# darchr/EmbeddingTables.jl

Measured on AMD Instinct MI355X. Metric: embedding lookups/sec + achieved HBM GB/s (% of roofline), 26 tables x dim128 at B=65536, higher is better.
Workload: dtype f32

## Files before the change

embeddingtables.jl_amd/csrc/et_lookup.hip:

```cpp
#include <type_traits>
#include "et_common.h"

#include <stdlib.h>
#include <string.h>

#include <mutex>
#include <utility>
#include <vector>

namespace et {

struct XcdQueue;
struct LookupPack {
    et_lookup_desc d[ET_MAX_TABLES_PER_LAUNCH];
    XcdQueue* queue = nullptr;
};

template <typename T, int D>
struct VecGeom {
    static constexpr int N = 16 / (int)sizeof(T);
    static constexpr int VPR = D / N;
    static constexpr int LPR = VPR < 64 ? VPR : 64;
    static constexpr int NV = VPR / LPR;
    static constexpr int GPW = 64 / LPR;
    static constexpr int U = NV >= 8 ? 1 : 8 / NV;
    static_assert(D % N == 0, "row must be whole vectors");
    static_assert(VPR <= 64 ? (64 % VPR == 0) : (VPR % 64 == 0), "unsupported row size");
};

template <typename T, int N>
__device__ __forceinline__ void unpack16(u32x4 v, T (&x)[N]) {
    static_assert(N * sizeof(T) == 16, "");
    __builtin_memcpy(x, &v, 16);
}

template <typename T, int N>
__device__ __forceinline__ u32x4 pack16(const T (&x)[N]) {
    u32x4 v;
    __builtin_memcpy(&v, x, 16);
    return v;
}

constexpr int kBcastReadlaneMaxGpw = 2;
template <int LPR>
__device__ __forceinline__ long long group_bcast(long long v, int i, int g) {
    constexpr int GPW = 64 / LPR;
    if constexpr (GPW <= kBcastReadlaneMaxGpw) {
        const int lo = (int)v, hi = (int)(v >> 32);
        int rlo = __builtin_amdgcn_readlane(lo, i), rhi = __builtin_amdgcn_readlane(hi, i);
#pragma unroll
        for (int gg = 1; gg < GPW; ++gg) {
            const int tlo = __builtin_amdgcn_readlane(lo, gg * LPR + i);
            const int thi = __builtin_amdgcn_readlane(hi, gg * LPR + i);
            rlo = g == gg ? tlo : rlo;
            rhi = g == gg ? thi : rhi;
        }
        return (long long)(((unsigned long long)(unsigned)rhi << 32) | (unsigned)rlo);
    } else {
        return __shfl(v, g * LPR + i, 64);
    }
}

template <int LPR>
__device__ __forceinline__ uint32_t group_bcast32(uint32_t v, int i, int g) {
    constexpr int GPW = 64 / LPR;
    if constexpr (GPW <= kBcastReadlaneMaxGpw) {
        int r = __builtin_amdgcn_readlane((int)v, i);
#pragma unroll
        for (int gg = 1; gg < GPW; ++gg) {
            const int t = __builtin_amdgcn_readlane((int)v, gg * LPR + i);
            r = g == gg ? t : r;
        }
        return (uint32_t)r;
    } else {
        return (uint32_t)__shfl((int)v, g * LPR + i, 64);
    }
}

__device__ __forceinline__ uint32_t idx_row32(long long v, uint32_t nrows) {
    const uint64_t row = (uint64_t)(v - 1);
    return row < (uint64_t)nrows ? (uint32_t)row : ~0u;
}

template <int LPR>
__device__ __forceinline__ long long load_idx_chunk(const int64_t* __restrict__ ip, int cnt,
                                                    int sub) {
    return (long long)ip[sub < cnt ? sub : cnt - 1];
}

template <typename T, typename A, int D, int UU, bool NTL, bool PG = false, bool MK = false>
__device__ __forceinline__ void load_add(const T* __restrict__ table, uint32_t ld_table,
                                         uint32_t nrows, uint32_t cpp, uint32_t myr, int g,
                                         int sub, int i0, bool first_batch,
                                         A (&acc)[VecGeom<T, D>::NV][VecGeom<T, D>::N],
                                         int& bad, int vpr) {
    using G = VecGeom<T, D>;
    constexpr int N = G::N, LPR = G::LPR, NV = G::NV;
    uint64_t off[UU];
    bool ok[UU];
    const T* base[UU];
#pragma unroll
    for (int u = 0; u < UU; ++u) {
        const uint32_t r = group_bcast32<LPR>(myr, i0 + u, g);
        ok[u] = r != ~0u;
        const uint32_t row32 = ok[u] ? r : 0u;
        if constexpr (PG) {
            const uint32_t page = row32 / cpp;
            off[u] = (uint64_t)(row32 - page * cpp) * ld_table;
            base[u] = reinterpret_cast<const T* const*>(table)[page];
        } else {
            off[u] = (uint64_t)row32 * ld_table;
            base[u] = table;
        }
    }
    int vix[NV];
#pragma unroll
    for (int v = 0; v < NV; ++v) {
        vix[v] = sub + v * LPR;
        if constexpr (MK) vix[v] = vix[v] < vpr ? vix[v] : vpr - 1;
    }
    u32x4 buf[UU][NV];
#pragma unroll
    for (int u = 0; u < UU; ++u) {
        const u32x4* src = reinterpret_cast<const u32x4*>(base[u] + off[u]);
#pragma unroll
        for (int v = 0; v < NV; ++v) {
            if constexpr (NTL)
                buf[u][v] = __builtin_nontemporal_load(src + vix[v]);
            else
                buf[u][v] = src[vix[v]];
        }
    }
    int anybad = 0;
#pragma unroll
    for (int u = 0; u < UU; ++u) anybad |= ok[u] ? 0 : 1;
    auto add_rows = [&](auto checked) {
#pragma unroll
        for (int u = 0; u < UU; ++u) {
#pragma unroll
            for (int v = 0; v < NV; ++v) {
                T x[N];
                if constexpr (decltype(checked)::value)
                    unpack16<T, N>(ok[u] ? buf[u][v] : u32x4{0u, 0u, 0u, 0u}, x);
                else
                    unpack16<T, N>(buf[u][v], x);
#pragma unroll
                for (int k = 0; k < N; ++k) {
                    if (u == 0)
                        acc[v][k] = first_batch ? A(x[k]) : A(acc[v][k] + A(x[k]));
                    else
                        acc[v][k] = A(acc[v][k] + A(x[k]));
                }
            }
        }
    };
    if (__builtin_expect(__any(anybad), 0)) {
#pragma unroll
        for (int u = 0; u < UU; ++u) bad += ok[u] ? 0 : 1;
        add_rows(std::true_type{});
    } else {
        add_rows(std::false_type{});
    }
}

template <typename T, typename A, int D, int U, bool NT, bool NTL, bool PG = false,
          bool MK = false>
__device__ __forceinline__ void bag_sum_vec(const T* __restrict__ table, uint32_t ld_table,
                                            uint32_t nrows, uint32_t cpp,
                                            const int64_t* __restrict__ ip,
                                            int pool, long long my0, T* __restrict__ out, int g,
                                            int sub, int vpr) {
    using G = VecGeom<T, D>;
    constexpr int N = G::N, LPR = G::LPR, NV = G::NV;
    A acc[NV][N];
#pragma unroll
    for (int v = 0; v < NV; ++v)
#pragma unroll
        for (int k = 0; k < N; ++k) acc[v][k] = A(0);
    int bad = 0;

    for (int c0 = 0; c0 < pool; c0 += LPR) {
        const int cnt = pool - c0 < LPR ? pool - c0 : LPR;
        const long long my = c0 == 0 ? my0 : load_idx_chunk<LPR>(ip + c0, cnt, sub);
        const uint32_t myr = idx_row32(my, nrows);
        int i0 = 0;
#define ET_LOAD_ADD(UU) \
    load_add<T, A, D, UU, NTL, PG, MK>(table, ld_table, nrows, cpp, myr, g, sub, i0,       \
                                       c0 + i0 == 0, acc, bad, vpr)
        for (; i0 + U <= cnt; i0 += U) ET_LOAD_ADD(U);
        if constexpr (U > 8) {
            if (cnt - i0 >= 8) {
                ET_LOAD_ADD(8);
                i0 += 8;
            }
        }
        if constexpr (U > 4) {
            if (cnt - i0 >= 4) {
                ET_LOAD_ADD(4);
                i0 += 4;
            }
        }
        if constexpr (U > 2) {
            if (cnt - i0 >= 2) {
                ET_LOAD_ADD(2);
                i0 += 2;
            }
        }
        if (cnt - i0 >= 1) ET_LOAD_ADD(1);
#undef ET_LOAD_ADD
    }
    if (bad && sub == 0) note_oob(bad);
    u32x4* o = reinterpret_cast<u32x4*>(out) + sub;
#pragma unroll
    for (int v = 0; v < NV; ++v) {
        T y[N];
#pragma unroll
        for (int k = 0; k < N; ++k) y[k] = T(acc[v][k]);
        if (!MK || sub + v * LPR < vpr) store16<NT>(o + v * LPR, pack16<T, N>(y));
    }
}

template <typename T, typename A, int D, int U, bool NT, bool NTL, bool PG = false,
          bool MK = false>
__device__ __forceinline__ void run_bags(const et_lookup_desc& d, int64_t batch,
                                         T* __restrict__ dst, int64_t ld_dst, int64_t chunk,
                                         int rounds) {
    using G = VecGeom<T, D>;
    const T* table = reinterpret_cast<const T*>(d.table);
    const int lane = threadIdx.x & 63, wave = threadIdx.x >> 6;
    const int g = lane / G::LPR, sub = lane % G::LPR;
    const int64_t per_round = 4 * G::GPW;
    const int pool = d.pool;
    const int cnt0 = pool < G::LPR ? pool : G::LPR;
    const uint32_t ldt = (uint32_t)d.ld_table, nr = (uint32_t)d.nrows;
    const int vpr = MK ? d.dim / G::N : G::VPR;
    int64_t bag = chunk * per_round * rounds + wave * G::GPW + g;
    long long my_next = load_idx_chunk<G::LPR>(
        d.idx + (bag < batch ? bag : batch - 1) * d.ld_idx, cnt0, sub);
    for (int r = 0; r < rounds; ++r) {
        if (bag >= batch) break;
        const long long my = my_next;
        const int64_t nbag = bag + per_round;
        if (r + 1 < rounds)
            my_next = load_idx_chunk<G::LPR>(
                d.idx + (nbag < batch ? nbag : batch - 1) * d.ld_idx, cnt0, sub);
        bag_sum_vec<T, A, D, U, NT, NTL, PG, MK>(table, ldt, nr, (uint32_t)d.cols_per_page,
                                                 d.idx + bag * d.ld_idx, pool, my,
                                                 dst + bag * ld_dst + d.dst_row_off, g, sub, vpr);
        bag = nbag;
    }
}

typedef const __attribute__((address_space(4))) int64_t* cidx_ptr;

__device__ __forceinline__ cidx_ptr as_scalar_idx(const int64_t* p) {
    return (cidx_ptr)(uintptr_t)p;
}

__device__ __forceinline__ uint64_t row_off_s(int64_t v, uint32_t ldb, uint32_t nrows,
                                              uint32_t& bad) {
    const uint32_t lo = (uint32_t)v - 1u;
    const uint32_t borrow = (uint32_t)(((uint64_t)lo - (uint64_t)nrows) >> 32);
    bad |= (uint32_t)((uint64_t)v >> 32) | ~borrow;
    return (((uint64_t)__umulhi(lo, ldb)) << 32) | (uint64_t)(lo * ldb);
}

template <typename T, typename A, int UU, bool NTL>
__device__ __forceinline__ bool load_add_s(uintptr_t tb, uint32_t ldb, uint32_t nrows,
                                           cidx_ptr ia, cidx_ptr ib, uint64_t hmask,
                                           uint64_t lane_off, bool first_batch,
                                           A (&acc)[16 / sizeof(T)]) {
    constexpr int N = 16 / (int)sizeof(T);
    typedef const __attribute__((address_space(1))) u32x4 gvec;
    uint64_t oa[UU], dd[UU];
    uint32_t bad = 0u;
#pragma unroll
    for (int u = 0; u < UU; ++u) {
        oa[u] = row_off_s(ia[u], ldb, nrows, bad);
        dd[u] = row_off_s(ib[u], ldb, nrows, bad) - oa[u];
    }
    if (bad) return false;
    u32x4 buf[UU];
#pragma unroll
    for (int u = 0; u < UU; ++u) {
        const uint64_t a = ((dd[u] & hmask) + lane_off) + (tb + oa[u]);
        const gvec* src = reinterpret_cast<const gvec*>(a);
        if constexpr (NTL)
            buf[u] = __builtin_nontemporal_load(src);
        else
            buf[u] = *src;
    }
#pragma unroll
    for (int u = 0; u < UU; ++u) {
        T x[N];
        __builtin_memcpy(x, &buf[u], 16);
#pragma unroll
        for (int k = 0; k < N; ++k) {
            if (u == 0)
                acc[k] = first_batch ? A(x[k]) : A(acc[k] + A(x[k]));
            else
                acc[k] = A(acc[k] + A(x[k]));
        }
    }
    return true;
}

template <typename T, typename A>
__device__ __forceinline__ void bag_pair_checked(uintptr_t tb, uint32_t ldb, uint32_t nrows,
                                                 const int64_t* ia, const int64_t* ib, bool hi,
                                                 int sub, int pool, A* acc, int* bad) {
    constexpr int N = 16 / (int)sizeof(T);
    const int64_t* ip = hi ? ib : ia;
#pragma unroll 1
    for (int i = 0; i < pool; ++i) {
        const uint64_t r = (uint64_t)(ip[i] - 1);
        const bool ok = r < (uint64_t)nrows;
        *bad += ok ? 0 : 1;
        const u32x4 v = *(reinterpret_cast<const u32x4*>(
                              tb + (uint64_t)(ok ? (uint32_t)r : 0u) * ldb) + sub);
        T x[N];
        unpack16<T, N>(ok ? v : u32x4{0u, 0u, 0u, 0u}, x);
        for (int k = 0; k < N; ++k) acc[k] = i == 0 ? A(x[k]) : A(acc[k] + A(x[k]));
    }
}

template <typename T, typename A, int U, bool NT, bool NTL>
__device__ __forceinline__ void run_bags_s(const et_lookup_desc& d, int64_t batch,
                                           T* __restrict__ dst, int64_t ld_dst, int64_t chunk,
                                           int rounds) {
    constexpr int N = 16 / (int)sizeof(T);
    const int lane = threadIdx.x & 63;
    const int wave = __builtin_amdgcn_readfirstlane(threadIdx.x >> 6);
    const bool hi = lane >= 32;
    const int sub = lane & 31;
    uint32_t hm = hi ? ~0u : 0u;
    asm volatile("" : "+v"(hm));
    const uint64_t hmask = ((uint64_t)hm << 32) | hm, lane_off = (uint64_t)sub * 16u;
    const uintptr_t tb = reinterpret_cast<uintptr_t>(d.table);
    const uint32_t ldb = (uint32_t)(d.ld_table * (int64_t)sizeof(T)), nr = (uint32_t)d.nrows;
    const int pool = d.pool;
    int64_t bag = chunk * 8 * rounds + 2 * wave;
    for (int r = 0; r < rounds; ++r, bag += 8) {
        if (bag >= batch) break;
        const bool has_b = bag + 1 < batch;
        const cidx_ptr ia = as_scalar_idx(d.idx + bag * d.ld_idx);
        const cidx_ptr ib = has_b ? as_scalar_idx(d.idx + (bag + 1) * d.ld_idx) : ia;
        A acc[N];
#pragma unroll
        for (int k = 0; k < N; ++k) acc[k] = A(0);
        bool ok = true;
        int i0 = 0;
#define ET_LOAD_ADD_S(UU) \
    load_add_s<T, A, UU, NTL>(tb, ldb, nr, ia + i0, ib + i0, hmask, lane_off, i0 == 0, acc)
        for (; ok && i0 + U <= pool; i0 += U) ok = ET_LOAD_ADD_S(U);
        if constexpr (U > 4) {
            if (ok && pool - i0 >= 4) {
                ok = ET_LOAD_ADD_S(4);
                i0 += 4;
            }
        }
        if constexpr (U > 2) {
            if (ok && pool - i0 >= 2) {
                ok = ET_LOAD_ADD_S(2);
                i0 += 2;
            }
        }
        if (ok && pool - i0 >= 1) ok = ET_LOAD_ADD_S(1);
#undef ET_LOAD_ADD_S
        int bad = 0;
        if (!ok)
            bag_pair_checked<T, A>(tb, ldb, nr, d.idx + bag * d.ld_idx,
                                   d.idx + (has_b ? bag + 1 : bag) * d.ld_idx, hi, sub, pool, acc,
                                   &bad);
        if (hi && !has_b) bad = 0;
        if (bad && sub == 0) note_oob(bad);
        if (!hi || has_b) {
            T y[N];
#pragma unroll
            for (int k = 0; k < N; ++k) y[k] = T(acc[k]);
            u32x4* o =
                reinterpret_cast<u32x4*>(dst + (bag + (hi ? 1 : 0)) * ld_dst + d.dst_row_off) + sub;
            store16<NT>(o, pack16<T, N>(y));
        }
    }
}

template <typename T, typename A, int D, int U, bool NT, bool PG = false, bool MK = false,
          bool SG = false>
__global__ __launch_bounds__(256) void k_pooled_vec(LookupPack pack, int ntables, int64_t batch,
                                                    T* __restrict__ dst, int64_t ld_dst,
                                                    int rounds) {
    const int64_t item = blockIdx.x;
    const int t = (int)(item % ntables);
    const int64_t chunk = item / ntables;
    if constexpr (SG)
        run_bags_s<T, A, U, NT, false>(pack.d[t], batch, dst, ld_dst, chunk, rounds);
    else
        run_bags<T, A, D, U, NT, false, PG, MK>(pack.d[t], batch, dst, ld_dst, chunk, rounds);
}

constexpr int kXcds = 8;

constexpr int kMaxStripeEntries = 40;
struct StripeMap {
    uint32_t entry[kXcds][kMaxStripeEntries];
    int nent;
    uint32_t ntload_mask;
    uint32_t prio_mask;
    int nheavy;
    int affinity;
    int fab_share;
};

template <typename T, typename A, int D, int U, bool NT, bool SG>
__device__ __forceinline__ void striped_body(const LookupPack& pack, const StripeMap& sm,
                                             int ntables, int64_t batch, T* __restrict__ dst,
                                             int64_t ld_dst, int rounds, int64_t stripe_chunks,
                                             int64_t nchunks, int x = blockIdx.x % kXcds,
                                             int64_t slot = blockIdx.x / kXcds) {
    const int k = (int)(slot % ntables);
    const int64_t j = slot / ntables;
    const uint32_t e = sm.entry[x][k];
    const int t = (int)(e & 0xff);
    const int64_t chunk = (int64_t)((e >> 8) & 0xff) * stripe_chunks + j;
    if (j >= stripe_chunks || chunk >= nchunks) return;
    if ((sm.prio_mask >> t) & 1u) __builtin_amdgcn_s_setprio(2);
    if constexpr (SG) {
        if ((sm.ntload_mask >> t) & 1u)
            run_bags_s<T, A, U, NT, true>(pack.d[t], batch, dst, ld_dst, chunk, rounds);
        else
            run_bags_s<T, A, U, NT, false>(pack.d[t], batch, dst, ld_dst, chunk, rounds);
    } else {
        if ((sm.ntload_mask >> t) & 1u)
            run_bags<T, A, D, U, NT, true>(pack.d[t], batch, dst, ld_dst, chunk, rounds);
        else
            run_bags<T, A, D, U, NT, false>(pack.d[t], batch, dst, ld_dst, chunk, rounds);
    }
}

#ifdef ET_WG_TIMELINE
constexpr uint32_t kTlCap = 1u << 17;
__device__ uint4 g_tl[kTlCap][2];
#endif

__device__ __forceinline__ uint64_t tl_begin() {
#ifdef ET_WG_TIMELINE
    return __builtin_amdgcn_s_memrealtime();
#else
    return 0;
#endif
}

__device__ __forceinline__ void tl_stamp(uint64_t t0, const StripeMap& sm, int ntables,
                                         int64_t stripe_chunks, int64_t nchunks, int x,
                                         int64_t slot) {
#ifdef ET_WG_TIMELINE
    __syncthreads();
    if (threadIdx.x == 0 && blockIdx.x < kTlCap) {
        const uint64_t t1 = __builtin_amdgcn_s_memrealtime();
        uint32_t xcc, hw;
        asm volatile("s_getreg_b32 %0, hwreg(HW_REG_XCC_ID)" : "=s"(xcc));
        asm volatile("s_getreg_b32 %0, hwreg(HW_REG_HW_ID)" : "=s"(hw));
        uint32_t t = 0xffu;
        if (x >= 0) {
            const int64_t j = slot / ntables;
            const uint32_t e = sm.entry[x][slot % ntables];
            const int64_t chunk = (int64_t)((e >> 8) & 0xff) * stripe_chunks + j;
            t = (j >= stripe_chunks || chunk >= nchunks ? 0xffu : (e & 0xffu)) | ((uint32_t)x << 8);
        }
        g_tl[blockIdx.x][0] = make_uint4((uint32_t)t0, (uint32_t)(t0 >> 32), (uint32_t)t1,
                                         (uint32_t)(t1 >> 32));
        g_tl[blockIdx.x][1] = make_uint4(t, xcc, hw, gridDim.x);
    }
#endif
}

template <typename T, typename A, int D, int U, bool NT, bool SG = false>
__global__ __launch_bounds__(256) void k_pooled_vec_striped(LookupPack pack, StripeMap sm,
                                                            int ntables, int64_t batch,
                                                            T* __restrict__ dst, int64_t ld_dst,
                                                            int rounds, int64_t stripe_chunks,
                                                            int64_t nchunks) {
    const uint64_t t0 = tl_begin();
    striped_body<T, A, D, U, NT, SG>(pack, sm, ntables, batch, dst, ld_dst, rounds, stripe_chunks,
                                     nchunks);
    tl_stamp(t0, sm, ntables, stripe_chunks, nchunks, blockIdx.x % kXcds, blockIdx.x / kXcds);
}

struct XcdQueue {
    uint32_t head[kXcds][2];
    uint32_t done;
    uint32_t pad[32 - 2 * kXcds - 1];
};
static_assert(sizeof(XcdQueue) == ET_LOOKUP_QUEUE_BYTES, "queue block size (include/embtab.h)");

__device__ __forceinline__ uint32_t cu_hash16(uint32_t hw) {
    const uint32_t cu = (hw >> 8) & 15u, sh = (hw >> 12) & 1u, se = (hw >> 13) & 7u;
    const uint32_t v = (cu + 3u * se + 5u * sh) & 15u;
    return ((v & 1u) << 3) | ((v & 2u) << 1) | ((v & 4u) >> 1) | ((v & 8u) >> 3);
}

__device__ __forceinline__ uint32_t claim_class(XcdQueue& q, uint32_t x, uint32_t c,
                                                uint32_t nheavy, uint32_t ntables, uint32_t sc) {
    const uint32_t nk = c ? ntables - nheavy : nheavy;
    const uint32_t h = atomicAdd(&q.head[x][c], 1u);
    if (h >= nk * sc) return ~0u;
    return x * (ntables * sc) + (h / nk) * ntables + (c ? nheavy : 0u) + h % nk;
}

__device__ __forceinline__ uint32_t claim_pref(XcdQueue& q, uint32_t x0, uint32_t p,
                                               uint32_t nheavy, uint32_t ntables, uint32_t sc) {
    constexpr uint32_t M = (uint32_t)(kXcds - 1);
    uint32_t it = claim_class(q, x0, p, nheavy, ntables, sc);
    if (it == ~0u && p == 1u) it = claim_class(q, x0, 0u, nheavy, ntables, sc);
    for (uint32_t k = 1; it == ~0u && k < (uint32_t)kXcds; ++k)
        it = claim_class(q, (x0 + k) & M, 0u, nheavy, ntables, sc);
    if (it == ~0u && p == 0u) it = claim_class(q, x0, 1u, nheavy, ntables, sc);
    for (uint32_t k = 1; it == ~0u && k < (uint32_t)kXcds; ++k)
        it = claim_class(q, (x0 + k) & M, 1u, nheavy, ntables, sc);
    return it;
}

template <typename T, typename A, int D, int U, bool NT, bool SG>
__global__ __launch_bounds__(256) void k_pooled_vec_queued(LookupPack pack, StripeMap sm,
                                                           int ntables, int64_t batch,
                                                           T* __restrict__ dst, int64_t ld_dst,
                                                           int rounds, int64_t stripe_chunks,
                                                           int64_t nchunks) {
    const uint64_t t0 = tl_begin();
    __shared__ uint32_t s_item;
    XcdQueue& q = *pack.queue;
    const uint32_t per = (uint32_t)(ntables * stripe_chunks);
    if (threadIdx.x == 0) {
        uint32_t xcc;
        asm volatile("s_getreg_b32 %0, hwreg(HW_REG_XCC_ID)" : "=s"(xcc));
        uint32_t it = ~0u;
        if (sm.affinity != 0) {
            const uint32_t x0 = xcc & (uint32_t)(kXcds - 1);
            const uint32_t nh = (uint32_t)sm.nheavy, sc = (uint32_t)stripe_chunks;
            uint32_t hw;
            asm volatile("s_getreg_b32 %0, hwreg(HW_REG_HW_ID)" : "=s"(hw));
            const uint32_t p = cu_hash16(hw) < (uint32_t)sm.fab_share ? 0u : 1u;
            it = claim_pref(q, x0, p, nh, (uint32_t)ntables, sc);
        } else
        for (uint32_t k = 0; k < (uint32_t)kXcds; ++k) {
            const uint32_t x = (xcc + k) & (uint32_t)(kXcds - 1);
            const uint32_t h = atomicAdd(&q.head[x][0], 1u);
            if (h < per) {
                it = x * per + h;
                break;
            }
        }
        s_item = it;
    }
    __syncthreads();
    const uint32_t it = s_item;
    if (it != ~0u)
        striped_body<T, A, D, U, NT, SG>(pack, sm, ntables, batch, dst, ld_dst, rounds,
                                         stripe_chunks, nchunks, (int)(it / per),
                                         (int64_t)(it % per));
    tl_stamp(t0, sm, ntables, stripe_chunks, nchunks, it != ~0u ? (int)(it / per) : -1,
             (int64_t)(it % per));
    if (threadIdx.x == 0 && atomicAdd(&q.done, 1u) == gridDim.x - 1u) {
        uint32_t* w = reinterpret_cast<uint32_t*>(&q);
        for (int i = 0; i < (int)(sizeof(XcdQueue) / sizeof(uint32_t)); ++i) atomicExch(&w[i], 0u);
    }
}

template <int RB, bool NT>
__global__ __launch_bounds__(256) void k_gather_vec(LookupPack pack, int ntables, int64_t batch,
                                                    char* __restrict__ dst, int64_t ld_dst_b,
                                                    int es, int rounds) {
    constexpr int VPR = RB / 16;
    constexpr int LPR = VPR < 64 ? VPR : 64;
    constexpr int NV = VPR / LPR;
    constexpr int GPW = 64 / LPR;
    constexpr int U = NV >= 8 ? 1 : 8 / NV;
    static_assert(VPR <= 64 ? (64 % VPR == 0) : (VPR % 64 == 0), "unsupported row size");

    const int64_t item = blockIdx.x;
    const int t = (int)(item % ntables);
    const int64_t chunk = item / ntables;
    const et_lookup_desc& d = pack.d[t];
    const char* table = reinterpret_cast<const char*>(d.table);
    const int64_t ld_b = d.ld_table * es;
    const int lane = threadIdx.x & 63, wave = threadIdx.x >> 6;
    const int g = lane / LPR, sub = lane % LPR;
    const int64_t per_round = 4 * GPW;
    const int64_t per_block = per_round * U * rounds;
    int64_t bag0 = chunk * per_block + wave * GPW + g;
    for (int r = 0; r < rounds; ++r, bag0 += per_round * U) {
        if (bag0 >= batch) break;
        uint64_t off[U];
        bool okv[U];
#pragma unroll
        for (int u = 0; u < U; ++u) {
            int64_t bag = bag0 + u * per_round;
            bag = bag < batch ? bag : batch - 1;
            const uint64_t row = (uint64_t)(d.idx[bag * d.ld_idx] - 1);
            okv[u] = row < (uint64_t)d.nrows;
            off[u] = okv[u] ? row * (uint64_t)ld_b : 0;
        }
        u32x4 buf[U][NV];
#pragma unroll
        for (int u = 0; u < U; ++u) {
            const u32x4* src = reinterpret_cast<const u32x4*>(table + off[u]) + sub;
#pragma unroll
            for (int v = 0; v < NV; ++v) buf[u][v] = src[v * LPR];
        }
        int bad = 0;
#pragma unroll
        for (int u = 0; u < U; ++u) {
            const int64_t bag = bag0 + u * per_round;
            if (bag < batch) {
                bad += okv[u] ? 0 : 1;
                u32x4* o =
                    reinterpret_cast<u32x4*>(dst + bag * ld_dst_b + d.dst_row_off * es) + sub;
#pragma unroll
                for (int v = 0; v < NV; ++v)
                    store16<NT>(o + v * LPR, okv[u] ? buf[u][v] : u32x4{0u, 0u, 0u, 0u});
            }
        }
        if (bad && sub == 0) note_oob(bad);
    }
}

template <int RB, bool NT, bool NTL, int U, int W = 4>
__global__ __launch_bounds__(64 * W) void k_gather_one(LookupPack pack, int ntables, int64_t batch,
                                                       char* __restrict__ dst, int64_t ld_dst_b,
                                                       int es) {
#ifdef ET_WG_TIMELINE
    const uint64_t tl0 = __builtin_amdgcn_s_memrealtime();
#endif
    constexpr int VPR = RB / 16;
    static_assert(VPR <= 64 && 64 % VPR == 0, "one vector per lane");
    constexpr int GPW = 64 / VPR;
    const int64_t item = blockIdx.x;
    const int t = (int)(item % ntables);
    const int64_t chunk = item / ntables;
    const et_lookup_desc& d = pack.d[t];
    const char* table = reinterpret_cast<const char*>(d.table);
    const int64_t ld_b = d.ld_table * es;
    const int lane = threadIdx.x & 63, wave = threadIdx.x >> 6;
    const int g = lane / VPR, sub = lane % VPR;
    const int64_t per_round = W * GPW;
    const int64_t bag0 = chunk * per_round * U + wave * GPW + g;
    int64_t iv[U];
#pragma unroll
    for (int u = 0; u < U; ++u) {
        int64_t b = bag0 + u * per_round;
        b = b < batch ? b : batch - 1;
        iv[u] = d.idx[b * d.ld_idx];
    }
    u32x4 cur[U];
    bool ok[U];
#pragma unroll
    for (int u = 0; u < U; ++u) {
        const uint64_t row = (uint64_t)(iv[u] - 1);
        ok[u] = row < (uint64_t)d.nrows;
        const u32x4* src = reinterpret_cast<const u32x4*>(table + (ok[u] ? row * (uint64_t)ld_b : 0)) + sub;
        if constexpr (NTL) cur[u] = __builtin_nontemporal_load(src);
        else cur[u] = *src;
    }
#ifdef ET_WG_TIMELINE
    asm volatile("" ::: "memory");
    const uint64_t tl1 = __builtin_amdgcn_s_memrealtime();
#endif
    int bad = 0;
#pragma unroll
    for (int u = 0; u < U; ++u) {
        const int64_t bag = bag0 + u * per_round;
        if (bag < batch) {
            bad += ok[u] ? 0 : 1;
            u32x4* o = reinterpret_cast<u32x4*>(dst + bag * ld_dst_b + d.dst_row_off * es) + sub;
            store16<NT>(o, ok[u] ? cur[u] : u32x4{0u, 0u, 0u, 0u});
        }
    }
    if (bad && sub == 0) note_oob(bad);
#ifdef ET_WG_TIMELINE
    asm volatile("s_waitcnt vmcnt(0)" ::: "memory");
    __syncthreads();
    if (threadIdx.x == 0 && blockIdx.x < kTlCap) {
        const uint64_t tl2 = __builtin_amdgcn_s_memrealtime();
        uint32_t xcc;
        asm volatile("s_getreg_b32 %0, hwreg(HW_REG_XCC_ID)" : "=s"(xcc));
        g_tl[blockIdx.x][0] = make_uint4((uint32_t)tl0, (uint32_t)(tl0 >> 32), (uint32_t)tl1,
                                         (uint32_t)(tl1 >> 32));
        g_tl[blockIdx.x][1] = make_uint4((uint32_t)tl2, (uint32_t)(tl2 >> 32), xcc, gridDim.x);
    }
#endif
}

template <typename O, typename T>
__device__ __forceinline__ O convert_elt(T x) {
    if constexpr ((__is_same(T, __bf16) || __is_same(O, __bf16)) && !__is_same(T, float) &&
                  !__is_same(O, float))
        return O((float)x);
    else
        return O(x);
}

template <typename T, typename A, bool NT, typename O = T>
__global__ __launch_bounds__(256) void k_pooled_generic(LookupPack pack, int ntables,
                                                        int64_t batch, O* __restrict__ dst,
                                                        int64_t ld_dst) {
    constexpr int K = 4;
    const int64_t item = blockIdx.x;
    const int t = (int)(item % ntables);
    const int64_t chunk = item / ntables;
    const et_lookup_desc& d = pack.d[t];
    const T* table = reinterpret_cast<const T*>(d.table);
    const int lane = threadIdx.x & 63, wave = threadIdx.x >> 6;
    const int64_t bag = chunk * 4 + wave;
    if (bag >= batch) return;
    const int64_t* ip = d.idx + bag * d.ld_idx;
    O* out = dst + bag * ld_dst + d.dst_row_off;
    const int dim = d.dim, pool = d.pool;
    for (int f0 = 0; f0 < dim; f0 += 64 * K) {
        A acc[K];
#pragma unroll
        for (int k = 0; k < K; ++k) acc[k] = A(0);
        for (int i = 0; i < pool; ++i) {
            uint64_t row = (uint64_t)(ip[i] - 1);
            const bool ok = row < (uint64_t)d.nrows;
            if (!ok && lane == 0 && f0 == 0) note_oob();
            row = ok ? row : 0;
            const T* src = col_ptr<const T>(d.table, d.ld_table, d.cols_per_page, row);
#pragma unroll
            for (int k = 0; k < K; ++k) {
                const int f = f0 + lane + 64 * k;
                if (f < dim) {
                    const T x = ok ? src[f] : T(0);
                    acc[k] = i == 0 ? A(x) : A(acc[k] + A(x));
                }
            }
        }
#pragma unroll
        for (int k = 0; k < K; ++k) {
            const int f = f0 + lane + 64 * k;
            if (f < dim) store_scalar<NT>(out + f, convert_elt<O>(T(acc[k])));
        }
    }
}


inline bool gather_rb_ok(int64_t rb) {
    return rb == 32 || rb == 64 || rb == 128 || rb == 256 || rb == 512 || rb == 1024 ||
           rb == 2048 || rb == 4096;
}

int max_rounds();

inline int rounds_for(int64_t batch, int64_t bags_per_round, int ntables) {
    int64_t blocks1 = (batch + bags_per_round - 1) / bags_per_round * ntables;
    int rounds = 1;
    const int mr = max_rounds();
    while (rounds < mr && blocks1 / (rounds * 2) >= 4096) rounds *= 2;
    return rounds;
}

struct LookupTuning {
    int striped = 1;
    int queued = 1;
    int ntload = 1;
    int64_t ntload_bytes = 256ll << 20;
    int max_rounds = 8;
    int64_t light_bytes = 4 << 20;
    int sgpr = 1;
    int heavy_prio = 0;
    int affinity = 1;
    int fab_share = 8;
};

inline const LookupTuning& tuning() {
    static LookupTuning t = [] {
        LookupTuning v;
#ifdef ET_EXPERIMENTS
        if (const char* e = getenv("ET_SCHED")) {
            v.striped = strcmp(e, "linear") != 0;
            v.queued = v.striped && strcmp(e, "stripe") != 0;
        }
        v.ntload = (int)ET_KNOB("ET_NTLOAD", v.ntload);
        v.ntload_bytes = ET_KNOB("ET_NTLOAD_BYTES", v.ntload_bytes);
        v.max_rounds = (int)ET_KNOB("ET_ROUNDS", v.max_rounds);
        if (v.max_rounds < 1) v.max_rounds = 1;
        v.light_bytes = ET_KNOB("ET_LIGHT_BYTES", v.light_bytes);
        v.sgpr = (int)ET_KNOB("ET_SGPR", v.sgpr);
        v.heavy_prio = (int)ET_KNOB("ET_HEAVY_PRIO", v.heavy_prio);
        if (const char* e = getenv("ET_AFFINITY")) v.affinity = *e == 'A' ? 1 : 0;
        v.fab_share = (int)ET_KNOB("ET_FAB_SHARE", v.fab_share);
#endif
        return v;
    }();
    return t;
}

int max_rounds() { return tuning().max_rounds; }

inline void build_stripe_map(const LookupPack& pack, int n, int es, StripeMap& sm) {
    const LookupTuning& tu = tuning();
    int heavy[ET_MAX_TABLES_PER_LAUNCH], light[ET_MAX_TABLES_PER_LAUNCH];
    int nh = 0, nl = 0;
    int64_t bytes[ET_MAX_TABLES_PER_LAUNCH];
    sm.ntload_mask = 0;
    sm.prio_mask = 0;
    for (int t = 0; t < n; ++t) {
        bytes[t] = pack.d[t].nrows * pack.d[t].ld_table * es;
        if (bytes[t] > tu.light_bytes) {
            heavy[nh++] = t;
            if (tu.heavy_prio) sm.prio_mask |= 1u << t;
            if (tu.ntload && bytes[t] > tu.ntload_bytes) sm.ntload_mask |= 1u << t;
        } else {
            light[nl++] = t;
        }
    }
    for (int a = 0; a < nl; ++a)
        for (int b = a + 1; b < nl; ++b)
            if (bytes[light[b]] > bytes[light[a]]) {
                int tmp = light[a];
                light[a] = light[b];
                light[b] = tmp;
            }
    int order[ET_MAX_TABLES_PER_LAUNCH];
    for (int i = 0, lo = 0, hi = nl - 1; i < nl; ++i) order[i] = (i & 1) ? light[hi--] : light[lo++];
    int cnt[kXcds] = {0};
    for (int x = 0; x < kXcds; ++x)
        for (int h = 0; h < nh; ++h) sm.entry[x][cnt[x]++] = (uint32_t)heavy[h] | ((uint32_t)x << 8);
    sm.nheavy = nh;
    for (int q = 0; q < nl * kXcds; ++q) {
        const int x = q / (nl > 0 ? nl : 1);
        sm.entry[x][cnt[x]++] = (uint32_t)order[q / kXcds] | ((uint32_t)(q % kXcds) << 8);
    }
    sm.nent = cnt[0];
    sm.affinity = sm.nheavy > 0 && sm.nheavy < sm.nent ? tu.affinity : 0;
    sm.fab_share = tu.fab_share < 0 ? 0 : tu.fab_share > 16 ? 16 : tu.fab_share;
    if (sm.fab_share == 0) sm.affinity = 0;
}

template <typename T, typename A, int D, bool NT, bool PG = false, bool MK = false>
int launch_pooled_vec(const LookupPack& pack, int n, int64_t batch, void* dst, int64_t ld_dst,
                      hipStream_t s) {
    using G = VecGeom<T, D>;
    constexpr int U = G::U;
    constexpr bool kSG = !PG && !MK && D * (int)sizeof(T) == 512;
    bool sg = kSG && tuning().sgpr;
    for (int t = 0; t < n && sg; ++t) sg = pack.d[t].ld_table * (int64_t)sizeof(T) < (1ll << 32);
    const int64_t per_round = sg ? 8 : 4 * G::GPW;
    const int rounds = rounds_for(batch, per_round, n);
    const int64_t nchunks = (batch + per_round * rounds - 1) / (per_round * rounds);
    if (nchunks <= 0) return ET_OK;
    const bool striped = !PG && !MK && n > 1 && tuning().striped;
    StripeMap sm;
    int64_t stripe_chunks = 0, grid = nchunks * n;
    if (striped) {
        build_stripe_map(pack, n, (int)sizeof(T), sm);
        stripe_chunks = (nchunks + kXcds - 1) / kXcds;
        grid = (int64_t)kXcds * sm.nent * stripe_chunks;
    }
    if (grid > 0x7fffffffll) return fail(ET_ERR_ARG, "grid too large");
    const bool queued = striped && pack.queue && tuning().queued;
    auto launch = [&](auto loop) -> int {
        constexpr bool SG = decltype(loop)::value;
        T* out = reinterpret_cast<T*>(dst);
        if constexpr (!PG && !MK) {
            if (queued) {
                hipLaunchKernelGGL((k_pooled_vec_queued<T, A, D, U, NT, SG>), dim3((unsigned)grid),
                                   dim3(256), 0, s, pack, sm, sm.nent, batch, out, ld_dst, rounds,
                                   stripe_chunks, nchunks);
                ET_LAUNCH_CHECK("k_pooled_vec_queued");
                return ET_OK;
            }
            if (striped) {
                hipLaunchKernelGGL((k_pooled_vec_striped<T, A, D, U, NT, SG>), dim3((unsigned)grid),
                                   dim3(256), 0, s, pack, sm, sm.nent, batch, out, ld_dst, rounds,
                                   stripe_chunks, nchunks);
                ET_LAUNCH_CHECK("k_pooled_vec_striped");
                return ET_OK;
            }
        }
        hipLaunchKernelGGL((k_pooled_vec<T, A, D, U, NT, PG, MK, SG>), dim3((unsigned)grid),
                           dim3(256), 0, s, pack, n, batch, out, ld_dst, rounds);
        ET_LAUNCH_CHECK("k_pooled_vec");
        return ET_OK;
    };
    if constexpr (kSG) {
        if (sg) return launch(std::true_type{});
    }
    return launch(std::false_type{});
}

template <int RB, bool NT>
int launch_gather_rb(const LookupPack& pack, int n, int64_t batch, void* dst, int64_t ld_dst,
                     int es, hipStream_t s) {
    constexpr int VPR = RB / 16;
    constexpr int LPR = VPR < 64 ? VPR : 64;
    constexpr int NV = VPR / LPR;
    constexpr int U = NV >= 8 ? 1 : 8 / NV;
    const int64_t per_round = 4 * (64 / LPR) * U;
    if constexpr (NV == 1 && U == 8) {
        bool ntl = tuning().ntload != 0;
        for (int t = 0; t < n && ntl; ++t)
            ntl = pack.d[t].nrows * pack.d[t].ld_table * es > tuning().ntload_bytes;
        constexpr int kU = 8, kW = 4;
        const int64_t pw = kW * (64 / LPR) * kU;
        const int64_t g1 = (batch + pw - 1) / pw * n;
        if (g1 <= 0) return ET_OK;
        if (g1 > 0x7fffffffll) return fail(ET_ERR_ARG, "grid too large");
        if (ntl)
            hipLaunchKernelGGL((k_gather_one<RB, NT, true, kU, kW>), dim3((unsigned)g1),
                               dim3(64 * kW), 0, s, pack, n, batch, reinterpret_cast<char*>(dst),
                               ld_dst * es, es);
        else
            hipLaunchKernelGGL((k_gather_one<RB, NT, false, kU, kW>), dim3((unsigned)g1),
                               dim3(64 * kW), 0, s, pack, n, batch, reinterpret_cast<char*>(dst),
                               ld_dst * es, es);
        ET_LAUNCH_CHECK("k_gather_one");
        return ET_OK;
    }
    const int rounds = rounds_for(batch, per_round, n);
    const int64_t nchunks = (batch + per_round * rounds - 1) / (per_round * rounds);
    const int64_t grid = nchunks * n;
    if (grid <= 0) return ET_OK;
    if (grid > 0x7fffffffll) return fail(ET_ERR_ARG, "grid too large");
    hipLaunchKernelGGL((k_gather_vec<RB, NT>), dim3((unsigned)grid), dim3(256), 0, s, pack, n,
                       batch, reinterpret_cast<char*>(dst), ld_dst * es, es, rounds);
    ET_LAUNCH_CHECK("k_gather_vec");
    return ET_OK;
}

template <bool NT>
int launch_gather(const LookupPack& pack, int n, int64_t rb, int64_t batch, void* dst,
                  int64_t ld_dst, int es, hipStream_t s) {
    switch (rb) {
        case 32: return launch_gather_rb<32, NT>(pack, n, batch, dst, ld_dst, es, s);
        case 64: return launch_gather_rb<64, NT>(pack, n, batch, dst, ld_dst, es, s);
        case 128: return launch_gather_rb<128, NT>(pack, n, batch, dst, ld_dst, es, s);
        case 256: return launch_gather_rb<256, NT>(pack, n, batch, dst, ld_dst, es, s);
        case 512: return launch_gather_rb<512, NT>(pack, n, batch, dst, ld_dst, es, s);
        case 1024: return launch_gather_rb<1024, NT>(pack, n, batch, dst, ld_dst, es, s);
        case 2048: return launch_gather_rb<2048, NT>(pack, n, batch, dst, ld_dst, es, s);
        case 4096: return launch_gather_rb<4096, NT>(pack, n, batch, dst, ld_dst, es, s);
    }
    return fail(ET_ERR_UNSUPPORTED, "gather row bytes %lld", (long long)rb);
}

template <typename T, typename A, bool NT, bool PG = false>
int launch_pooled_dim(const LookupPack& pack, int n, int D, int64_t batch, void* dst,
                      int64_t ld_dst, hipStream_t s) {
    switch (D) {
        case 16: return launch_pooled_vec<T, A, 16, NT, PG>(pack, n, batch, dst, ld_dst, s);
        case 32: return launch_pooled_vec<T, A, 32, NT, PG>(pack, n, batch, dst, ld_dst, s);
        case 64: return launch_pooled_vec<T, A, 64, NT, PG>(pack, n, batch, dst, ld_dst, s);
        case 128: return launch_pooled_vec<T, A, 128, NT, PG>(pack, n, batch, dst, ld_dst, s);
        case 256: return launch_pooled_vec<T, A, 256, NT, PG>(pack, n, batch, dst, ld_dst, s);
        case 512: return launch_pooled_vec<T, A, 512, NT, PG>(pack, n, batch, dst, ld_dst, s);
    }
    return fail(ET_ERR_UNSUPPORTED, "vector dim %d", D);
}

template <typename T, typename A, bool NT>
int launch_pooled_masked(const LookupPack& pack, int n, int D, int64_t batch, void* dst,
                         int64_t ld_dst, hipStream_t s) {
#define ET_MK(C)                                                                              \
    case C:                                                                                   \
        if constexpr (C / (16 / (int)sizeof(T)) >= 1)                                         \
            return launch_pooled_vec<T, A, C, NT, false, true>(pack, n, batch, dst, ld_dst,   \
                                                               s);                            \
        break;
    switch (masked_capacity(D)) {
        ET_MK(16)
        ET_MK(32)
        ET_MK(64)
        ET_MK(128)
        ET_MK(256)
        ET_MK(512)
        ET_MK(1024)
        ET_MK(2048)
    }
#undef ET_MK
    return fail(ET_ERR_UNSUPPORTED, "masked vector dim %d", D);
}

template <typename T, typename A, bool NT>
int launch_generic(const LookupPack& pack, int n, int64_t batch, void* dst, int64_t ld_dst,
                   hipStream_t s) {
    const int64_t grid = (batch + 3) / 4 * n;
    if (grid <= 0) return ET_OK;
    if (grid > 0x7fffffffll) return fail(ET_ERR_ARG, "grid too large");
    hipLaunchKernelGGL((k_pooled_generic<T, A, NT>), dim3((unsigned)grid), dim3(256), 0, s, pack,
                       n, batch, reinterpret_cast<T*>(dst), ld_dst);
    ET_LAUNCH_CHECK("k_pooled_generic");
    return ET_OK;
}

enum GroupKind { kGather = 0, kPooledVec = 1, kGeneric = 2, kPagedVec = 3, kMaskedVec = 4 };

template <typename T, typename A, bool NT>
int launch_group_typed(GroupKind kind, const LookupPack& pack, int n, int D, int64_t batch,
                       void* dst, int64_t ld_dst, hipStream_t s) {
    const int es = (int)sizeof(T);
    if (kind == kGather)
        return launch_gather<NT>(pack, n, (int64_t)D * es, batch, dst, ld_dst, es, s);
    if (kind == kPooledVec) return launch_pooled_dim<T, A, NT>(pack, n, D, batch, dst, ld_dst, s);
    if (kind == kPagedVec)
        return launch_pooled_dim<T, A, NT, true>(pack, n, D, batch, dst, ld_dst, s);
    if (kind == kMaskedVec)
        return launch_pooled_masked<T, A, NT>(pack, n, D, batch, dst, ld_dst, s);
    return launch_generic<T, A, NT>(pack, n, batch, dst, ld_dst, s);
}

template <bool NT>
int launch_group(int dtype, bool f32acc, GroupKind kind, const LookupPack& pack, int n, int D,
                 int64_t batch, void* dst, int64_t ld_dst, hipStream_t s) {
    switch (dtype) {
        case ET_F32:
            return launch_group_typed<float, float, NT>(kind, pack, n, D, batch, dst, ld_dst, s);
        case ET_F64:
            return launch_group_typed<double, double, NT>(kind, pack, n, D, batch, dst, ld_dst, s);
        case ET_I32:
            return launch_group_typed<int32_t, uint32_t, NT>(kind, pack, n, D, batch, dst, ld_dst,
                                                            s);
        case ET_I64:
            return launch_group_typed<int64_t, uint64_t, NT>(kind, pack, n, D, batch, dst, ld_dst,
                                                            s);
        case ET_BF16:
            return launch_group_typed<__bf16, float, NT>(kind, pack, n, D, batch, dst, ld_dst,
                                                         s);
        case ET_F16:
            if (f32acc)
                return launch_group_typed<_Float16, float, NT>(kind, pack, n, D, batch, dst,
                                                               ld_dst, s);
            return launch_group_typed<_Float16, _Float16, NT>(kind, pack, n, D, batch, dst, ld_dst,
                                                              s);
    }
    return fail(ET_ERR_UNSUPPORTED, "dtype %d", dtype);
}

int validate_lookup(const et_lookup_desc* descs, int ntables, int64_t batch, const void* dst,
                    int64_t ld_dst) {
    if (ntables < 0 || batch < 0) return fail(ET_ERR_ARG, "negative ntables/batch");
    if (ntables == 0 || batch == 0) return 1;
    if (!descs) return fail(ET_ERR_ARG, "descs is NULL");
    if (!dst) return fail(ET_ERR_ARG, "dst is NULL");
    for (int t = 0; t < ntables; ++t) {
        const et_lookup_desc& d = descs[t];
        if (d.dim < 0 || d.pool < 0 || d.nrows < 0 || d.cols_per_page < 0)
            return fail(ET_ERR_ARG, "table %d: negative dim/pool/nrows/cols_per_page", t);
        if (d.dim == 0) continue;
        if (d.ld_table < d.dim) return fail(ET_ERR_ARG, "table %d: ld_table < dim", t);
        if (d.dst_row_off < 0 || d.dst_row_off + d.dim > ld_dst)
            return fail(ET_ERR_ARG, "table %d: rows [%lld, %lld) outside ld_dst %lld", t,
                        (long long)d.dst_row_off, (long long)(d.dst_row_off + d.dim),
                        (long long)ld_dst);
        if (d.pool > 0) {
            if (!d.table || !d.idx) return fail(ET_ERR_ARG, "table %d: NULL table/idx", t);
            if (d.nrows == 0)
                return fail(ET_ERR_ARG, "table %d: indices into an empty table", t);
            if (d.ld_idx < d.pool) return fail(ET_ERR_ARG, "table %d: ld_idx < pool", t);
        }
    }
    return ET_OK;
}

int lookup_dispatch(int dtype, const et_lookup_desc* descs, int ntables, int64_t batch,
                    void* dst, int64_t ld_dst, uint32_t flags, hipStream_t s,
                    void* queue = nullptr) {
    const int es = elsize(dtype);
    if (es == 0) return fail(ET_ERR_UNSUPPORTED, "unknown dtype %d", dtype);
    const int v = validate_lookup(descs, ntables, batch, dst, ld_dst);
    if (v != ET_OK) return v == 1 ? ET_OK : v;
    const bool nt = (flags & ET_FLAG_NONTEMPORAL) != 0;
    const bool f32acc = (flags & ET_FLAG_F16_FP32_ACC) != 0;

    int kind_of[4096];
    if (ntables > 4096) return fail(ET_ERR_ARG, "too many tables (%d)", ntables);
    for (int t = 0; t < ntables; ++t) {
        const et_lookup_desc& d = descs[t];
        const bool al = aligned16(d.table) && ((d.ld_table * es) % 16 == 0) &&
                        aligned16(static_cast<char*>(dst) + d.dst_row_off * es) &&
                        ((ld_dst * es) % 16 == 0);
        if (d.dim == 0) {
            kind_of[t] = -1;
        } else if (d.cols_per_page != 0) {
            const bool vec = d.pool >= 1 && al && vec_dim_ok(d.dim) && d.nrows < 0xffffffffll &&
                             d.ld_table < 0xffffffffll && d.cols_per_page < 0xffffffffll;
            kind_of[t] = vec ? kPagedVec : kGeneric;
        } else if (d.pool == 1 && al && gather_rb_ok((int64_t)d.dim * es)) {
            kind_of[t] = kGather;
        } else if (d.pool >= 1 && al && vec_dim_ok(d.dim) && d.nrows < 0xffffffffll &&
                   d.ld_table < 0xffffffffll) {
            kind_of[t] = kPooledVec;
        } else if (d.pool >= 1 && al && ((int64_t)d.dim * es) % 16 == 0 && d.dim <= 2048 &&
                   d.nrows < 0xffffffffll && d.ld_table < 0xffffffffll) {
            kind_of[t] = kMaskedVec;
        } else {
            kind_of[t] = kGeneric;
        }
    }
    bool done[4096] = {false};
    for (int t0 = 0; t0 < ntables; ++t0) {
        if (done[t0] || kind_of[t0] < 0) continue;
        LookupPack pack;
        pack.queue = static_cast<XcdQueue*>(queue);
        int n = 0;
        const GroupKind kind = (GroupKind)kind_of[t0];
        const int D = descs[t0].dim;
        for (int t = t0; t < ntables; ++t) {
            if (done[t] || kind_of[t] != kind_of[t0]) continue;
            if (kind != kGeneric && descs[t].dim != D) continue;
            pack.d[n++] = descs[t];
            done[t] = true;
            if (n == ET_MAX_TABLES_PER_LAUNCH) {
                int rc = nt ? launch_group<true>(dtype, f32acc, kind, pack, n, D, batch, dst,
                                                 ld_dst, s)
                            : launch_group<false>(dtype, f32acc, kind, pack, n, D, batch, dst,
                                                  ld_dst, s);
                if (rc != ET_OK) return rc;
                n = 0;
            }
        }
        if (n > 0) {
            int rc = nt ? launch_group<true>(dtype, f32acc, kind, pack, n, D, batch, dst, ld_dst, s)
                        : launch_group<false>(dtype, f32acc, kind, pack, n, D, batch, dst,
                                              ld_dst, s);
            if (rc != ET_OK) return rc;
        }
    }
    return ET_OK;
}

template <typename T, typename A, typename O>
int launch_convert(const et_lookup_desc* descs, int ntables, int64_t batch, void* dst,
                   int64_t ld_dst, bool nt, hipStream_t s) {
    for (int t0 = 0; t0 < ntables; t0 += ET_MAX_TABLES_PER_LAUNCH) {
        LookupPack pack;
        int n = 0;
        for (int t = t0; t < ntables && n < ET_MAX_TABLES_PER_LAUNCH; ++t) pack.d[n++] = descs[t];
        const int64_t grid = (batch + 3) / 4 * n;
        if (grid > 0x7fffffffll) return fail(ET_ERR_ARG, "grid too large");
        if (nt)
            hipLaunchKernelGGL((k_pooled_generic<T, A, true, O>), dim3((unsigned)grid), dim3(256),
                               0, s, pack, n, batch, reinterpret_cast<O*>(dst), ld_dst);
        else
            hipLaunchKernelGGL((k_pooled_generic<T, A, false, O>), dim3((unsigned)grid),
                               dim3(256), 0, s, pack, n, batch, reinterpret_cast<O*>(dst), ld_dst);
        ET_LAUNCH_CHECK("k_pooled_generic");
    }
    return ET_OK;
}

template <typename T, typename A>
int convert_to(int out_dtype, const et_lookup_desc* descs, int ntables, int64_t batch, void* dst,
               int64_t ld_dst, bool nt, hipStream_t s) {
    switch (out_dtype) {
        case ET_F32: return launch_convert<T, A, float>(descs, ntables, batch, dst, ld_dst, nt, s);
        case ET_F64: return launch_convert<T, A, double>(descs, ntables, batch, dst, ld_dst, nt, s);
        case ET_F16:
            return launch_convert<T, A, _Float16>(descs, ntables, batch, dst, ld_dst, nt, s);
        case ET_BF16:
            return launch_convert<T, A, __bf16>(descs, ntables, batch, dst, ld_dst, nt, s);
    }
    return fail(ET_ERR_UNSUPPORTED, "destination dtype %d", out_dtype);
}
// ... 123 lines not shown
```

Baseline: 28.12 billion.

## Reorder queued stripe claims per XCD to table-major cache-friendly order

Moves stripe placement into a new header and adds per-XCD claim-order policies for the queued kernel. For the light (cached) class, entries are sorted largest-first and claimed table-major, so consecutive blocks on an XCD work through one table's chunks before moving on, which should improve L2/MALL reuse. For the heavy class, policy fab=3 rotates the heavy tables per XCD and also claims them table-major, so different XCDs begin on different heavy tables. This adds a small per-claim index computation and a larger kernel argument struct, and changes load balance across XCDs.

Result: faster. 29.42 billion (median of 6 runs) (+4.6%).

```diff
diff --git a/embeddingtables.jl_amd/csrc/et_lookup.hip b/embeddingtables.jl_amd/csrc/et_lookup.hip
--- a/embeddingtables.jl_amd/csrc/et_lookup.hip
+++ b/embeddingtables.jl_amd/csrc/et_lookup.hip
@@ -1,5 +1,6 @@
 #include <type_traits>
 #include "et_common.h"
+#include "et_lookup_order.h"
 
 #include <stdlib.h>
 #include <string.h>
@@ -400,8 +401,10 @@
 }
 
 constexpr int kXcds = 8;
-
-constexpr int kMaxStripeEntries = 40;
+static_assert(kXcds == et_order::kXcds && ET_MAX_TABLES_PER_LAUNCH == et_order::kMaxTables,
+              "et_lookup_order.h");
+
+constexpr int kMaxStripeEntries = et_order::kMaxEntries;
 struct StripeMap {
     uint32_t entry[kXcds][kMaxStripeEntries];
     int nent;
@@ -410,6 +413,7 @@
     int nheavy;
     int affinity;
     int fab_share;
+    et_order::ClassOrder order[2];
 };
 
 template <typename T, typename A, int D, int U, bool NT, bool SG>
@@ -500,24 +504,25 @@
     return ((v & 1u) << 3) | ((v & 2u) << 1) | ((v & 4u) >> 1) | ((v & 8u) >> 3);
 }
 
-__device__ __forceinline__ uint32_t claim_class(XcdQueue& q, uint32_t x, uint32_t c,
-                                                uint32_t nheavy, uint32_t ntables, uint32_t sc) {
-    const uint32_t nk = c ? ntables - nheavy : nheavy;
+__device__ __forceinline__ uint32_t claim_class(XcdQueue& q, const StripeMap& sm, uint32_t x,
+                                                uint32_t c, uint32_t nheavy, uint32_t ntables,
+                                                uint32_t sc) {
     const uint32_t h = atomicAdd(&q.head[x][c], 1u);
-    if (h >= nk * sc) return ~0u;
-    return x * (ntables * sc) + (h / nk) * ntables + (c ? nheavy : 0u) + h % nk;
-}
-
-__device__ __forceinline__ uint32_t claim_pref(XcdQueue& q, uint32_t x0, uint32_t p,
-                                               uint32_t nheavy, uint32_t ntables, uint32_t sc) {
+    const uint32_t slot = et_order::class_slot(sm.order[c], x, c, h, nheavy, ntables, sc);
+    return slot == et_order::kNone ? ~0u : x * (ntables * sc) + slot;
+}
+
+__device__ __forceinline__ uint32_t claim_pref(XcdQueue& q, const StripeMap& sm, uint32_t x0,
+                                               uint32_t p, uint32_t nheavy, uint32_t ntables,
+                                               uint32_t sc) {
     constexpr uint32_t M = (uint32_t)(kXcds - 1);
-    uint32_t it = claim_class(q, x0, p, nheavy, ntables, sc);
-    if (it == ~0u && p == 1u) it = claim_class(q, x0, 0u, nheavy, ntables, sc);
+    uint32_t it = claim_class(q, sm, x0, p, nheavy, ntables, sc);
+    if (it == ~0u && p == 1u) it = claim_class(q, sm, x0, 0u, nheavy, ntables, sc);
     for (uint32_t k = 1; it == ~0u && k < (uint32_t)kXcds; ++k)
-        it = claim_class(q, (x0 + k) & M, 0u, nheavy, ntables, sc);
-    if (it == ~0u && p == 0u) it = claim_class(q, x0, 1u, nheavy, ntables, sc);
+        it = claim_class(q, sm, (x0 + k) & M, 0u, nheavy, ntables, sc);
+    if (it == ~0u && p == 0u) it = claim_class(q, sm, x0, 1u, nheavy, ntables, sc);
     for (uint32_t k = 1; it == ~0u && k < (uint32_t)kXcds; ++k)
-        it = claim_class(q, (x0 + k) & M, 1u, nheavy, ntables, sc);
+        it = claim_class(q, sm, (x0 + k) & M, 1u, nheavy, ntables, sc);
     return it;
 }
 
@@ -541,7 +546,7 @@
             uint32_t hw;
             asm volatile("s_getreg_b32 %0, hwreg(HW_REG_HW_ID)" : "=s"(hw));
             const uint32_t p = cu_hash16(hw) < (uint32_t)sm.fab_share ? 0u : 1u;
-            it = claim_pref(q, x0, p, nh, (uint32_t)ntables, sc);
+            it = claim_pref(q, sm, x0, p, nh, (uint32_t)ntables, sc);
         } else
         for (uint32_t k = 0; k < (uint32_t)kXcds; ++k) {
             const uint32_t x = (xcc + k) & (uint32_t)(kXcds - 1);
@@ -770,6 +775,7 @@
     int heavy_prio = 0;
     int affinity = 1;
     int fab_share = 8;
+    et_order::Policy order = {1, 3, 1 << 20};
 };
 
 inline const LookupTuning& tuning() {
@@ -789,6 +795,9 @@
         v.heavy_prio = (int)ET_KNOB("ET_HEAVY_PRIO", v.heavy_prio);
         if (const char* e = getenv("ET_AFFINITY")) v.affinity = *e == 'A' ? 1 : 0;
         v.fab_share = (int)ET_KNOB("ET_FAB_SHARE", v.fab_share);
+        v.order.cache_major = (int)ET_KNOB("ET_ORDER_CACHE", v.order.cache_major);
+        v.order.fab = (int)ET_KNOB("ET_ORDER_FAB", v.order.fab);
+        v.order.phase_bytes = ET_KNOB("ET_PHASE_BYTES", v.order.phase_bytes);
 #endif
         return v;
     }();
@@ -797,44 +806,27 @@
 
 int max_rounds() { return tuning().max_rounds; }
 
-inline void build_stripe_map(const LookupPack& pack, int n, int es, StripeMap& sm) {
+inline void build_stripe_map(const LookupPack& pack, int n, int es, bool queued, StripeMap& sm) {
     const LookupTuning& tu = tuning();
-    int heavy[ET_MAX_TABLES_PER_LAUNCH], light[ET_MAX_TABLES_PER_LAUNCH];
-    int nh = 0, nl = 0;
     int64_t bytes[ET_MAX_TABLES_PER_LAUNCH];
     sm.ntload_mask = 0;
     sm.prio_mask = 0;
     for (int t = 0; t < n; ++t) {
         bytes[t] = pack.d[t].nrows * pack.d[t].ld_table * es;
         if (bytes[t] > tu.light_bytes) {
-            heavy[nh++] = t;
             if (tu.heavy_prio) sm.prio_mask |= 1u << t;
             if (tu.ntload && bytes[t] > tu.ntload_bytes) sm.ntload_mask |= 1u << t;
-        } else {
-            light[nl++] = t;
-        }
-    }
-    for (int a = 0; a < nl; ++a)
-        for (int b = a + 1; b < nl; ++b)
-            if (bytes[light[b]] > bytes[light[a]]) {
-                int tmp = light[a];
-                light[a] = light[b];
-                light[b] = tmp;
-            }
-    int order[ET_MAX_TABLES_PER_LAUNCH];
-    for (int i = 0, lo = 0, hi = nl - 1; i < nl; ++i) order[i] = (i & 1) ? light[hi--] : light[lo++];
-    int cnt[kXcds] = {0};
-    for (int x = 0; x < kXcds; ++x)
-        for (int h = 0; h < nh; ++h) sm.entry[x][cnt[x]++] = (uint32_t)heavy[h] | ((uint32_t)x << 8);
-    sm.nheavy = nh;
-    for (int q = 0; q < nl * kXcds; ++q) {
-        const int x = q / (nl > 0 ? nl : 1);
-        sm.entry[x][cnt[x]++] = (uint32_t)order[q / kXcds] | ((uint32_t)(q % kXcds) << 8);
-    }
-    sm.nent = cnt[0];
+        }
+    }
+    sm.nent = et_order::place_stripes(bytes, n, tu.light_bytes, sm.entry, &sm.nheavy);
     sm.affinity = sm.nheavy > 0 && sm.nheavy < sm.nent ? tu.affinity : 0;
     sm.fab_share = tu.fab_share < 0 ? 0 : tu.fab_share > 16 ? 16 : tu.fab_share;
     if (sm.fab_share == 0) sm.affinity = 0;
+    memset(sm.order, 0, sizeof(sm.order));
+    if (queued && sm.affinity != 0)
+        for (int x = 0; x < kXcds; ++x)
+            et_order::order_xcd(sm.entry[x], x, sm.nent, sm.nheavy, bytes, sm.ntload_mask, tu.order,
+                                sm.order);
 }
 
 template <typename T, typename A, int D, bool NT, bool PG = false, bool MK = false>
@@ -852,13 +844,13 @@
     const bool striped = !PG && !MK && n > 1 && tuning().striped;
     StripeMap sm;
     int64_t stripe_chunks = 0, grid = nchunks * n;
+    const bool queued = striped && pack.queue && tuning().queued;
     if (striped) {
-        build_stripe_map(pack, n, (int)sizeof(T), sm);
+        build_stripe_map(pack, n, (int)sizeof(T), queued, sm);
         stripe_chunks = (nchunks + kXcds - 1) / kXcds;
         grid = (int64_t)kXcds * sm.nent * stripe_chunks;
     }
     if (grid > 0x7fffffffll) return fail(ET_ERR_ARG, "grid too large");
-    const bool queued = striped && pack.queue && tuning().queued;
     auto launch = [&](auto loop) -> int {
         constexpr bool SG = decltype(loop)::value;
         T* out = reinterpret_cast<T*>(dst);
diff --git a/embeddingtables.jl_amd/csrc/et_lookup_order.h b/embeddingtables.jl_amd/csrc/et_lookup_order.h
--- /dev/null
+++ b/embeddingtables.jl_amd/csrc/et_lookup_order.h
@@ -0,0 +1,153 @@
+#pragma once
+#include <stdint.h>
+
+#if defined(__HIPCC__) || defined(__CUDACC__)
+#define ET_ORDER_FN __host__ __device__ inline
+#else
+#define ET_ORDER_FN inline
+#endif
+
+namespace et_order {
+
+constexpr int kXcds = 8;
+constexpr uint32_t kNone = ~0u;
+constexpr uint32_t kTablesFastest = 0, kTableMajor = 1;
+
+struct ClassOrder {
+    uint8_t split[kXcds];
+    uint8_t major[kXcds];
+};
+
+ET_ORDER_FN uint32_t class_slot(uint32_t h, uint32_t nk, uint32_t base, uint32_t ntables,
+                                uint32_t sc, uint32_t split, uint32_t major0, uint32_t major1) {
+    if (h >= nk * sc) return kNone;
+    if (split > nk) split = nk;
+    uint32_t n = split, first = 0, major = major0;
+    if (h >= split * sc) {
+        h -= split * sc;
+        n = nk - split;
+        first = split;
+        major = major1;
+    }
+    const uint32_t j = major == kTableMajor ? h % sc : h / n;
+    const uint32_t k = major == kTableMajor ? h / sc : h % n;
+    return j * ntables + base + first + k;
+}
+
+ET_ORDER_FN uint32_t class_slot(const ClassOrder& o, uint32_t x, uint32_t c, uint32_t h,
+                                uint32_t nheavy, uint32_t ntables, uint32_t sc) {
+    const uint32_t nk = c ? ntables - nheavy : nheavy;
+    return class_slot(h, nk, c ? nheavy : 0u, ntables, sc, o.split[x], o.major[x] & 1u,
+                      (o.major[x] >> 1) & 1u);
+}
+
+
+constexpr int kMaxEntries = 40;
+constexpr int kMaxTables = 32;
+
+inline uint32_t entry_table(uint32_t e) { return e & 0xffu; }
+
+inline int place_stripes(const int64_t* table_bytes, int n, int64_t light_bytes,
+                         uint32_t entry[][kMaxEntries], int* nheavy) {
+    int heavy[kMaxTables], light[kMaxTables];
+    int nh = 0, nl = 0;
+    for (int t = 0; t < n; ++t)
+        if (table_bytes[t] > light_bytes) heavy[nh++] = t;
+        else light[nl++] = t;
+    for (int a = 0; a < nl; ++a)
+        for (int b = a + 1; b < nl; ++b)
+            if (table_bytes[light[b]] > table_bytes[light[a]]) {
+                int tmp = light[a];
+                light[a] = light[b];
+                light[b] = tmp;
+            }
+    int order[kMaxTables];
+    for (int i = 0, lo = 0, hi = nl - 1; i < nl; ++i) order[i] = (i & 1) ? light[hi--] : light[lo++];
+    int cnt[kXcds] = {0};
+    for (int x = 0; x < kXcds; ++x)
+        for (int h = 0; h < nh; ++h) entry[x][cnt[x]++] = (uint32_t)heavy[h] | ((uint32_t)x << 8);
+    for (int q = 0; q < nl * kXcds; ++q) {
+        const int x = q / (nl > 0 ? nl : 1);
+        entry[x][cnt[x]++] = (uint32_t)order[q / kXcds] | ((uint32_t)(q % kXcds) << 8);
+    }
+    *nheavy = nh;
+    return cnt[0];
+}
+
+
+template <typename F>
+inline int stable_front(uint32_t* e, int n, F first) {
+    uint32_t tmp[256];
+    int a = 0, b = 0;
+    for (int i = 0; i < n; ++i)
+        if (first(e[i])) e[a++] = e[i];
+        else tmp[b++] = e[i];
+    for (int i = 0; i < b; ++i) e[a + i] = tmp[i];
+    return a;
+}
+
+inline void rotate_left(uint32_t* e, int n, int r) {
+    if (n <= 1) return;
+    uint32_t tmp[256];
+    for (int i = 0; i < n; ++i) tmp[i] = e[(i + r) % n];
+    for (int i = 0; i < n; ++i) e[i] = tmp[i];
+}
+
+inline void largest_first(uint32_t* e, int n, const int64_t* table_bytes) {
+    for (int i = 1; i < n; ++i) {
+        const uint32_t v = e[i];
+        int k = i;
+        for (; k > 0 && table_bytes[entry_table(e[k - 1])] < table_bytes[entry_table(v)]; --k)
+            e[k] = e[k - 1];
+        e[k] = v;
+    }
+}
+
+inline int64_t class_footprint(const uint32_t* e, int n, const int64_t* table_bytes) {
+    uint32_t seen = 0;
+    int64_t sum = 0;
+    for (int i = 0; i < n; ++i) {
+        const uint32_t t = entry_table(e[i]);
+        if (!((seen >> t) & 1u)) sum += table_bytes[t];
+        seen |= 1u << t;
+    }
+    return sum;
+}
+
+inline int two_phases(uint32_t* e, int n, uint32_t nt_mask, bool nt_first, int rot) {
+    const int nnt =
+        stable_front(e, n, [&](uint32_t v) { return ((nt_mask >> entry_table(v)) & 1u) != 0; });
+    const int nal = n - nnt;
+    if (nal > 0) rotate_left(e + nnt, nal, rot % nal);
+    if (nt_first) return nnt;
+    rotate_left(e, n, nnt);
+    return nal;
+}
+
+struct Policy {
+    int cache_major = 0;
+    int fab = 0;
+    int64_t phase_bytes = 1 << 20;
+};
+
+inline void order_xcd(uint32_t* e, int x, int ntables, int nheavy, const int64_t* table_bytes,
+                      uint32_t nt_mask, const Policy& p, ClassOrder ord[2]) {
+    uint32_t* ce = e + nheavy;
+    const int nc = ntables - nheavy;
+    ord[0].split[x] = ord[1].split[x] = 0;
+    ord[0].major[x] = ord[1].major[x] = 0;
+    if (p.cache_major) {
+        largest_first(ce, nc, table_bytes);
+        ord[1].major[x] = 3;
+    }
+    if (p.fab == 1 || p.fab == 2) {
+        const bool nt_first = class_footprint(ce, nc, table_bytes) > p.phase_bytes;
+        ord[0].split[x] = (uint8_t)two_phases(e, nheavy, nt_mask, nt_first, p.fab == 2 ? x : 0);
+        if (p.fab == 2) ord[0].major[x] = nt_first ? 2 : 1;
+    } else if (p.fab == 3) {
+        rotate_left(e, nheavy, nheavy > 0 ? x % nheavy : 0);
+        ord[0].major[x] = 3;
+    }
+}
+
+}
```
